# nanoporetech/vbz_compression

Hardware: AMD Instinct MI355X
Metric: MB/s encode+decode, int16 signal, 1/2/4/8 MI355X vs CPU; ratio preserved (higher is better)
Workload: dtype int16

## Files before the change

### vbz_compression_amd/csrc/vbz_api.hip

```cpp
#include <hip/hip_runtime.h>

#include <cmath>
#include <cstdarg>
#include <cstdio>
#include <cstdlib>
#include <cstring>
#include <condition_variable>
#include <mutex>
#include <string>
#include <map>
#include <vector>

#include "../../include/vbz.h"
#include "../../include/vbz_gpu.h"
#include "vbz_kernels.h"

using namespace vbzhip;


struct ProfEntry
{
    const char* name;
    uint32_t launches;
    double ms;
// ... 152 lines not shown

void drain_profile(vbz_gpu_ctx* c)
{
    if (c->pending.empty()) return;
    (void)hipStreamSynchronize(c->stream);
    for (auto& p : c->pending) {
        float ms = 0;
        (void)hipEventElapsedTime(&ms, p.start, p.stop);
        bool found = false;
        for (auto& e : c->prof)
            if (e.name == p.name || strcmp(e.name, p.name) == 0) {
                e.launches++;
                e.ms += ms;
                found = true;
                break;
            }
        if (!found) c->prof.push_back({ p.name, 1, (double)ms });
        c->event_pool.push_back(p.start);
        c->event_pool.push_back(p.stop);
    }
    c->pending.clear();
}

unsigned long long* dbg_begin(vbz_gpu_ctx* c, uint32_t n)
{
    if (!c->phase_timing) return nullptr;
    if (!ensure(c, c->dbg, (size_t)n * PHASE_SLOTS * 8)) return nullptr;
    (void)hipMemsetAsync(c->dbg.p, 0, (size_t)n * PHASE_SLOTS * 8, c->stream);
    return (unsigned long long*)c->dbg.p;
}

void dbg_end(vbz_gpu_ctx* c, uint32_t n, const char* what, unsigned long long* d)
{
    if (!d) return;
    std::vector<unsigned long long> h((size_t)n * PHASE_SLOTS);
    (void)hipStreamSynchronize(c->stream);
    (void)hipMemcpy(h.data(), d, (size_t)n * PHASE_SLOTS * 8, hipMemcpyDeviceToHost);
    double sum[PHASE_SLOTS] = {};
    for (uint32_t i = 0; i < n; ++i)
        for (int k = 0; k < PHASE_SLOTS; ++k) sum[k] += (double)h[(size_t)i * PHASE_SLOTS + k];
    fprintf(stderr, "vbz_hip phase cycles/read (%s, n=%u):", what, n);
    for (int k = 0; k < PHASE_SLOTS; ++k) fprintf(stderr, " p%d=%.0f", k, sum[k] / n);
    fprintf(stderr, "\n");
}

bool half_codec(const CompressionOptions* o) { return o->vbz_version == 1 && o->integer_size == 1; }

bool pod5_codec(const CompressionOptions* o) { return o->vbz_version == VBZ_GPU_VERSION_POD5; }

bool valid_int_size(const CompressionOptions* o)
{
    return o->integer_size == 0 || o->integer_size == 1 || o->integer_size == 2 || o->integer_size == 4;
}

bool batch_options_ok(const CompressionOptions* o, int sized)
{
    if (pod5_codec(o)) return o->integer_size == 2 && o->perform_delta_zig_zag && o->zstd_compression_level >= 1 && sized == 0;
// ... 205 lines not shown
            gate = pre->gate;
            scratch_planned = true;
        }
    }
    void* const scratch_base = pre ? pre->scratch : c->scratch.p;
    const ScratchPlan splan = { num, den, c->scratch.cap, svb_off, svb_cap, gate };
    if (segmented && plan_segments(c, n, bt->src_size, rb_in.gate, bt->src_bytes, svb_seg_unit_bytes((int)o->integer_size), &seg,
                                   both_stages ? &splan : nullptr, &scratch_planned) != 0)
        return -1;
    if (segmented) rb.gate = seg.gate;
    if (o->integer_size != 0 && o->zstd_compression_level == 0) {
        Timed t(c, "svb_encode");
        if (segmented)
            HIPCHK(c, launch_svb_encode_seg(rb, (int)o->integer_size, o->perform_delta_zig_zag, hdr, true, seg.first, seg.max_segs, seg.val, seg.off, s),
                   "svb_encode (segmented) launch");
        else
            HIPCHK(c, launch_svb_encode(rb, (int)o->integer_size, o->perform_delta_zig_zag, hdr, true, half_codec(o), nullptr, nullptr, s), "svb_encode launch");
        return 0;
    }
    if (o->integer_size == 0) {
        if (checksum_content(c, rb, rb.gate) != 0) return -1;
        {
            Timed t(c, "zstd_encode");
            HIPCHK(c, launch_zstd_encode(rb, bt->src_size, 0, nullptr, hdr, nullptr, nullptr, nullptr, c->trailers, nullptr, nullptr, false, false, nullptr, s), "zstd_encode launch");
        }
        return checksum_frames(c, rb, rb.gate, hdr, bt->src_size, 0);
    }
    const bool matcher = !segmented && c->zero_run_sequences && c->long_repeats;
    if (!scratch_planned) {
        if (rb.gate) HIPCHK(c, hipMemcpyAsync(gate, rb.gate, 4ull * n, hipMemcpyDeviceToDevice, s), "gate copy");
        Timed t(c, "plan_scratch");
        HIPCHK(c, launch_plan_scratch(n, bt->src_size, num, den, c->scratch.cap, svb_off, svb_cap, gate, rb.gate != nullptr, s), "plan launch");
    }
    ReadBatch a = rb;
    a.dst = (uint8_t*)scratch_base;
    a.dst_off = svb_off;
    a.dst_cap = svb_cap;
    a.result = svb_size;
    a.gate = gate;
    unsigned long long* dbg = segmented ? nullptr : dbg_begin(c, n);
    const bool staged = !segmented && c->staged_encode && (!dbg || c->phase_timing == 3) && c->zero_run_sequences;
    const bool pod5 = pod5_codec(o);
    const bool pre_filled = staged && !pod5 && svb_encode_fills_plans((int)o->integer_size, o->perform_delta_zig_zag, half_codec(o));
    void* plan = nullptr;
    if (staged) {
        if (!ensure(c, c->encplan, zstd_encode_plan_bytes(n))) return -1;
        plan = c->encplan.p;
    }
    const uint32_t* key_orig = bt->src_size;
    uint32_t key_elem = o->integer_size;
    if (pod5) {
        HIPCHK(c, launch_svb16_key_raw(n, bt->src_size, key_raw, s), "svb16 key launch");
        key_orig = key_raw;
        key_elem = SVB16_KEY_ELEM;
    }
    {
        Timed t(c, "svb_encode");
        if (pod5)
            HIPCHK(c, launch_svb16_encode(a, (matcher && !segmented) ? deep_d : nullptr, s), "svb16_encode launch");
        else if (segmented)
            HIPCHK(c, launch_svb_encode_seg(a, (int)o->integer_size, o->perform_delta_zig_zag, 0, false, seg.first, seg.max_segs, seg.val, seg.off, s),
                   "svb_encode (segmented) launch");
        else
            HIPCHK(c, launch_svb_encode(a, (int)o->integer_size, o->perform_delta_zig_zag, 0, false, half_codec(o), matcher ? deep_d : nullptr,
// ... 22 lines not shown
        uint32_t* span_first = sm.take<uint32_t>((size_t)n + 1);
        uint32_t* span_count = sm.take<uint32_t>(1);
        uint32_t* span_size = sm.take<uint32_t>(max_spans);
        uint32_t* span_trail = sm.take<uint32_t>(max_spans);
        uint32_t* span_dst = sm.take<uint32_t>(max_spans);
        z.gate = gate;
        if (c->zero_run_sequences && c->long_repeats && o->integer_size != 0) {
            uint32_t* gate2 = mc.take<uint32_t>(n);
            Timed t(c, "zstd_encode_matcher");
            HIPCHK(c, launch_zstd_encode_matcher(z, key_orig, key_elem, hdr, svb_cap, c->seqtab.p, c->trailers, 0xFFFFFFFFu,
                                                 deep_d, gate, gate2, s),
                   "zstd_encode (matcher) launch");
            z.gate = gate2;
        }
        Timed t(c, "zstd_encode");
        HIPCHK(c, launch_zstd_encode_spans(z, key_orig, key_elem, hdr, c->zero_run_sequences ? svb_cap : nullptr,
                                           c->zero_run_sequences ? c->seqtab.p : nullptr, desc, span_first, span_count, max_spans,
                                           (uint8_t*)c->spantmp.p, tmp_bytes, span_size, span_trail, span_dst, c->trailers, regions, shspan, s),
               "zstd_encode (spans) launch");
        return checksum_frames(c, z, gate, hdr, pod5 ? nullptr : bt->src_size, o->integer_size);
    }
    {
        Timed t(c, "zstd_encode");
        HIPCHK(c, launch_zstd_encode(z, key_orig, key_elem, nullptr, hdr, c->phase_timing == 3 ? nullptr : dbg,
                                     c->zero_run_sequences ? svb_cap : nullptr, c->zero_run_sequences ? c->seqtab.p : nullptr, c->trailers,
                                     (matcher && !dbg) ? deep_d : nullptr, plan, staged, pre_filled, c->phase_timing == 3 ? dbg : nullptr, s),
               "zstd_encode launch");
    }
    dbg_end(c, n,
            c->phase_timing == 3   ? "zstd_pack: setup region lookups+scan bits quads ends+headers sequences trailer"
            : c->phase_timing == 2 ? "zstd_encode planning launch: setup hist plan - store+sequences - | plan: sort merge lengths codes weights tree"
                                   : "zstd_encode: setup hist plan size hdr encode",
            dbg);
    return checksum_frames(c, z, gate, hdr, pod5 ? nullptr : bt->src_size, o->integer_size);
}

constexpr uint32_t REF_MIN_READS = 2560;

int zstd_frames(vbz_gpu_ctx* c, const ReadBatch& z, uint32_t toosmall_code, uint64_t content_bytes, unsigned long long* dbg)
{
    const uint32_t n = z.n_reads;
    hipStream_t s = c->stream;
    Timed t(c, "zstd_decode");
    c->last_frames = 0;
    if (!c->fast_decode) {
        HIPCHK(c, launch_zstd_decode(z, toosmall_code, dbg, c->seqdtab.p, s), "zstd_decode launch");
        return 0;
    }
    if (!ensure(c, c->fastmeta, zstd_fast_meta_bytes(n))) return -1;
    const bool walk = (c->ref_chains >= 2 || (c->ref_chains == 1 && n >= REF_MIN_READS)) && (c->foreign_state != 0 || c->ref_chains >= 2);
    const uint64_t recs_bytes = walk ? std::min<uint64_t>(((content_bytes >> 2) + (1ull << 20)) & ~15ull, 1ull << 30) : 0;
    if (walk && (!ensure(c, c->refpre, zstd_ref_pre_bytes(n)) || !ensure(c, c->reftab, zstd_ref_table_bytes(n)) || !ensure(c, c->refrecs, recs_bytes)))
        return -1;
    if (walk && !dbg && !ensure_side(c)) return -1;
    const bool lits = walk && zstd_ref_literals_enabled();
    if (lits && !ensure(c, c->reflits, zstd_ref_lit_meta_bytes(n))) return -1;
// ... 914 lines not shown
        if (integer_size != 2 || !zigzag) return -2;
        Timed t(c, "svb_decode");
        HIPCHK(c, launch_svb16_decode(to_rb(bt), c->stream), "svb16_decode launch");
        return 0;
    }
    if ((integer_size != 1 && integer_size != 2 && integer_size != 4) || version > 1 || version < 0) return -2;
    Timed t(c, "svb_decode");
    HIPCHK(c, launch_svb_decode(to_rb(bt), integer_size, zigzag != 0, version == 1 && integer_size == 1, c->stream), "svb_decode launch");
    return 0;
}

uint64_t vbz_gpu_pod5_max_compressed_size(uint32_t samples)
{
    const uint64_t n = samples, svb = (n + 7) / 8 + 2 * n;
    return svb + (svb >> 8) + (svb < (128u << 10) ? (((128u << 10) - svb) >> 11) : 0);
}

int vbz_gpu_zstd_compress_batch(vbz_gpu_ctx* c, const vbz_gpu_batch* bt, const uint32_t* key_bytes)
{
    if (!c || !bt) return -1;
    DeviceGuard dg(c->device);
    if (checksum_content(c, to_rb(bt), nullptr) != 0) return -1;
    Timed t(c, "zstd_encode");
    HIPCHK(c, launch_zstd_encode(to_rb(bt), bt->src_size, 0, key_bytes, 0, nullptr, nullptr, nullptr, c->trailers, nullptr, nullptr, false, false, nullptr, c->stream), "zstd_encode launch");
    return checksum_frames(c, to_rb(bt), nullptr, 0, nullptr, 0);
}

int vbz_gpu_zstd_decompress_batch(vbz_gpu_ctx* c, const vbz_gpu_batch* bt)
{
    if (!c || !bt) return -1;
    DeviceGuard dg(c->device);
    if (!plausible_extents(c, bt)) return -2;
    if (zstd_frames(c, to_rb(bt), E_ZSTD, bt->dst_bytes, nullptr) != 0) return -1;
    return verify_checksums(c, to_rb(bt));
}

int vbz_gpu_xxh64_batch(vbz_gpu_ctx* c, const vbz_gpu_batch* bt, uint64_t* out)
{
    if (!c || !bt || !out) return -1;
    DeviceGuard dg(c->device);
    Timed t(c, "xxh64");
    HIPCHK(c, launch_xxh64_batch((const uint8_t*)bt->src, bt->src_off, bt->src_size, nullptr, nullptr, bt->n_reads, out, c->stream), "xxh64 launch");
    return 0;
}

static bool pack_align_ok(vbz_gpu_ctx* c, uint32_t align)
{
// ... 573 lines not shown
```

### vbz_compression_amd/csrc/vbz_kernels.h

```cpp
#pragma once

#include <hip/hip_runtime.h>
#include <stdint.h>

namespace vbzhip {

constexpr uint32_t E_ZSTD = 0xFFFFFFFFu;
constexpr uint32_t E_INPUT_SIZE = 0xFFFFFFFEu;
constexpr uint32_t E_INTEGER_SIZE = 0xFFFFFFFDu;
constexpr uint32_t E_DESTINATION_SIZE = 0xFFFFFFFCu;
constexpr uint32_t E_STREAM = 0xFFFFFFFBu;
constexpr uint32_t E_VERSION = 0xFFFFFFFAu;
constexpr uint32_t E_OOM = 0xFFFFFFF9u;
constexpr uint32_t E_DEVICE = 0xFFFFFFF8u;
constexpr uint32_t E_FIRST = E_DEVICE;
constexpr uint32_t GATE_SKIP = E_FIRST - 1u;
constexpr int PHASE_SLOTS = 12;

constexpr uint32_t SIG_NONE = 0, SIG_F32 = 1, SIG_F16 = 2, SIG_BF16 = 3;
constexpr uint32_t SIG_CHUNK = 4;
constexpr uint32_t SIG_COUNT = 8;
constexpr uint32_t CHUNK_PAD = 0, CHUNK_END = 1;

constexpr uint32_t NORM_MED_MAD = 1, NORM_QUANTILE = 2;
// ... 78 lines not shown
    uint32_t pad[8];
    uint32_t histB[256];
};
constexpr uint32_t PLAN_OPEN = 1, PLAN_REG0 = 2, PLAN_REG1 = 4, PLAN_READY = 7;
constexpr uint32_t ENC_TRAILERS = 1, ENC_PRE_FILLED = 2;
inline EncPlan* zstd_encode_plans(void* plan_meta) { return reinterpret_cast<EncPlan*>(plan_meta); }

hipError_t launch_svb_encode(const ReadBatch& b, int integer_size, bool zigzag, uint32_t hdr, bool strict_cap, bool half, uint32_t* period_hint,
                             void* plans, hipStream_t s);
bool svb_encode_fills_plans(int integer_size, bool zigzag, bool half);
hipError_t launch_svb_decode(const ReadBatch& b, int integer_size, bool zigzag, bool half, hipStream_t s);
hipError_t launch_svb16_encode(const ReadBatch& b, uint32_t* period_hint, hipStream_t s);
hipError_t launch_svb16_decode(const ReadBatch& b, hipStream_t s);
hipError_t launch_svb16_key_raw(uint32_t n, const uint32_t* raw_size, uint32_t* key_raw, hipStream_t s);
constexpr uint32_t SVB16_KEY_ELEM = 4;
uint32_t svb_seg_unit_bytes(int integer_size);
hipError_t launch_svb_encode_seg(const ReadBatch& b, int integer_size, bool zigzag, uint32_t hdr, bool strict_cap, const uint32_t* seg_first,
                                 uint32_t max_segs, uint32_t* seg_bytes, uint64_t* seg_off, hipStream_t s);
hipError_t launch_svb_decode_seg(const ReadBatch& b, int integer_size, bool zigzag, const uint32_t* seg_first, uint32_t max_segs,
                                 uint32_t* seg_val, uint64_t* seg_pos, uint32_t* seg_run, hipStream_t s);

hipError_t launch_zstd_encode(const ReadBatch& b, const uint32_t* orig_size, uint32_t key_elem, const uint32_t* key_bytes,
                              uint32_t hdr, unsigned long long* dbg, const uint32_t* src_cap, const void* seq_tables, bool trailers,
                              uint32_t* deep_d, void* plan_meta, bool staged, bool pre_filled, unsigned long long* pack_dbg, hipStream_t s);
size_t zstd_encode_plan_bytes(uint32_t n_reads);
size_t seq_tables_bytes();
void seq_tables_build(void* host_buffer);
struct SideStream
{
    hipStream_t stream = nullptr;
    hipEvent_t fork = nullptr, join = nullptr;
};
typedef SideStream FastSide;
size_t zstd_span_desc_bytes();
uint32_t zstd_span_max_spans(uint64_t stream_bytes, uint32_t n_reads);
uint64_t zstd_span_tmp_bytes(uint64_t stream_bytes, uint32_t n_reads, uint32_t max_spans);
hipError_t launch_zstd_encode_spans(const ReadBatch& b, const uint32_t* orig_size, uint32_t key_elem, uint32_t hdr, const uint32_t* src_cap,
                                    const void* seq_tables, void* span_desc, uint32_t* span_first, uint32_t* span_count, uint32_t max_spans,
                                    uint8_t* span_tmp, uint64_t span_tmp_bytes, uint32_t* span_size, uint32_t* span_trail, uint32_t* span_dst,
                                    bool trailers, void* shared_regions, uint32_t shared_span_bytes, hipStream_t s);
size_t zstd_span_region_bytes(uint32_t n_reads);
uint32_t zstd_span_shared_bytes(uint64_t stream_bytes);
hipError_t launch_zstd_encode_matcher(const ReadBatch& b, const uint32_t* orig_size, uint32_t key_elem, uint32_t hdr, const uint32_t* src_cap,
                                      const void* seq_tables, bool trailers, uint32_t max_raw, uint32_t* deep_d, const uint32_t* gate_in,
                                      uint32_t* gate_out, hipStream_t s);
hipError_t launch_zstd_decode(const ReadBatch& b, uint32_t toosmall_code, unsigned long long* dbg, const void* seq_dtables,
                              hipStream_t s);
// ... 163 lines not shown
```

### vbz_compression_amd/csrc/zstd_encode.hip

```cpp
#include "vbz_kernels.h"
#include "zstd_entropy.h"
#include "zstd_frame.h"

namespace vbzhip {

namespace {

constexpr int WAVE = 64;
constexpr uint32_t BLOCK_MAX = 128u << 10;
constexpr uint32_t MIN_BLOCK = 4096;
constexpr uint32_t HUF_BLOCK_MAX = 92u << 10;
constexpr uint32_t SPLIT_MIN = 2048;
constexpr int MAXBLK = 16;
#ifndef VBZ_SPAN_BLOCK_KB
#define VBZ_SPAN_BLOCK_KB 16
#endif
constexpr uint32_t SPAN_BLOCK = VBZ_SPAN_BLOCK_KB << 10;
#ifndef VBZ_SPAN_SMALL_BLOCKS
#define VBZ_SPAN_SMALL_BLOCKS 2
#endif
constexpr uint32_t SPAN_BYTES_SMALL = SPAN_BLOCK * VBZ_SPAN_SMALL_BLOCKS, SPAN_BYTES_LARGE = SPAN_BLOCK * MAXBLK;
constexpr uint32_t SPAN_LARGE_FROM = 256u << 20;
#ifndef VBZ_KEYSPAN_KB
#define VBZ_KEYSPAN_KB 8
// ... 57 lines not shown
    uint32_t mode;
    uint32_t huffLog;
    uint32_t rankcnt[16];
    union
    {
        HufPmWksp pm;
        FseWeightWksp fw;
        struct
        {
            uint32_t ssize[WAVE];
            uint32_t sbeg[WAVE];
            uint32_t scnt[WAVE];
            uint32_t obuf[OBUF_WORDS];
            uint16_t seqcode[8 + 256];
            uint32_t seqpiece[256];
        };
    };
    SeqCTables seq;
    uint32_t cp[64];
    uint32_t cpCount, cpSpacing;
    __device__ __forceinline__ void set_code(uint32_t s, uint32_t code, uint32_t nb) { ctable[s] = make_uint2(code, nb); }
};

struct TableLds
{
    uint32_t hist[256];
    uint32_t ctable[256];
    uint8_t nbBits[256];
    uint8_t weights[260];
    uint8_t tree[136];
    int32_t treeSize;
    uint32_t mode;
    uint32_t huffLog;
    uint32_t rankcnt[16];
    union
    {
        HufPmWksp pm;
        FseWeightWksp fw;
    };
    __device__ __forceinline__ void set_code(uint32_t s, uint32_t code, uint32_t nb) { ctable[s] = code | (nb << 16); }
};
struct TokSeqLds
{
    uint32_t obuf[128];
    uint16_t seqcode[8 + 256];
    uint32_t seqpiece[256];
    SeqCTables seq;
    uint32_t cp[64];
    uint32_t cpCount, cpSpacing;
};

__device__ __forceinline__ void put_le(uint8_t* p, uint64_t v, int n)
{
    for (int i = 0; i < n; ++i) {
        uint32_t byte = (uint32_t)(v >> (8 * i)) & 0xFFu;
        asm volatile("" : "+v"(byte));
        p[i] = (uint8_t)byte;
    }
}

__device__ __forceinline__ uint32_t wave_sum_u32(uint32_t v)
// ... 35 lines not shown
{
    uint32_t seen = 0;
    uint32_t c[4];
#pragma unroll
    for (int j = 0; j < 4; ++j) {
        c[j] = sample[lane + 64 * j];
        seen += c[j] ? 1u : 0u;
    }
    seen = wave_sum_u32(seen);
    if (allow_sample && n >= HIST_SAMPLE_FROM && seen >= HIST_SAMPLE_SEEN) {
#pragma unroll
        for (int j = 0; j < 4; ++j) L.hist[lane + 64 * j] = c[j] ? c[j] : 1u;
        wave_lds_sync();
        return hist_sample_bytes(in, n) + (256u - seen);
    }
    if (!rest) return region_histogram(L, in, n, lane, allow_sample);
#pragma unroll
    for (int j = 0; j < 4; ++j) L.hist[lane + 64 * j] = c[j] + rest[lane + 64 * j];
    wave_lds_sync();
    return n;
}

template <class LDS>
__device__ __forceinline__ uint32_t region_histogram(LDS& L, const uint8_t* in, uint32_t n, int lane, bool allow_sample)
{
    static_assert(sizeof(HufPmWksp) >= 4 * 256 * sizeof(uint32_t), "the sub-histograms live in the table-construction workspace");
    uint32_t* sub = reinterpret_cast<uint32_t*>(&L.pm);
    for (int i = lane; i < 4 * 256; i += WAVE) sub[i] = 0;
    wave_lds_sync();
    uint32_t* mine = sub + 256 * (lane & 3);
    const uint32_t head = (uint32_t)((16u - ((uintptr_t)in & 15u)) & 15u);
    const uint32_t h = head < n ? head : n;
    if ((uint32_t)lane < h) atomicAdd(&mine[in[lane]], 1u);
    const uint32_t nvec = (n - h) >> 4;
    const uint4* vp = reinterpret_cast<const uint4*>(in + h);
    const uint32_t tail0 = h + (nvec << 4);
    if (tail0 + (uint32_t)lane < n) atomicAdd(&mine[in[tail0 + lane]], 1u);
    auto count = [&](uint32_t first_stripe, uint32_t stripe_step, uint32_t trip_stripes, int loads) {
        for (uint32_t s0 = first_stripe; s0 * WAVE < nvec; s0 += trip_stripes) {
            uint4 q[4];
#pragma unroll
            for (int u = 0; u < 4; ++u) {
                const uint32_t c = (s0 + (uint32_t)u * stripe_step) * WAVE + (uint32_t)lane;
                q[u] = (u < loads && c < nvec) ? vp[c] : make_uint4(0u, 0u, 0u, 0u);
            }
#pragma unroll
            for (int u = 0; u < 4; ++u) {
                const uint32_t c = (s0 + (uint32_t)u * stripe_step) * WAVE + (uint32_t)lane;
                if (u < loads && c < nvec) {
                    const uint32_t w[4] = { q[u].x, q[u].y, q[u].z, q[u].w };
// ... 30 lines not shown
        count(1, 1, 4, 3);
    } else {
        count(0, 1, 4, 4);
    }
    (void)total();
    return n;
}

#define SUB(k) do { if (tsub) { unsigned long long tn = __builtin_readcyclecounter(); tsub[k] += tn - *tl; *tl = tn; } } while (0)
template <bool STRICT>
__device__ __forceinline__ uint32_t sorted_count(const uint32_t* arr, uint32_t v, uint32_t top)
{
    uint32_t lo = 0;
    for (uint32_t step = top; step; step >>= 1) {
        const uint32_t x = arr[lo + step - 1];
        lo += (STRICT ? x < v : x <= v) ? step : 0u;
    }
    return lo;
}

template <class LDS>
__device__ __forceinline__ uint32_t huf_build_wave(LDS& L, uint32_t maxSym, uint32_t maxNbBits, int lane, unsigned long long* tsub = nullptr, unsigned long long* tl = nullptr)
{
    HufPmWksp& K = L.pm;
    uint32_t key[4];
    {
        const uint4 h = *reinterpret_cast<const uint4*>(&L.hist[4 * lane]);
        const uint32_t c[4] = { h.x, h.y, h.z, h.w };
#pragma unroll
        for (int j = 0; j < 4; ++j) {
            const uint32_t sy = 4u * (uint32_t)lane + (uint32_t)j;
            key[j] = (sy <= maxSym && c[j]) ? ((c[j] << 8) | (255u - sy)) : 0xFFFFFFFFu;
        }
    }
    for (int i = lane; i < (HUF_MAX_BITS + 1) * 16; i += WAVE) (&K.isPkg[0][0])[i] = 0;
#pragma unroll
    for (int k = 2; k <= 256; k <<= 1) {
#pragma unroll
        for (int d = k >> 1; d > 0; d >>= 1) {
            if (d >= 4) {
                const int m = d >> 2;
                const bool up = ((4 * lane) & k) == 0, lower = (lane & m) == 0;
                const bool keep_min = lower == up;
#pragma unroll
                for (int j = 0; j < 4; ++j) {
                    const uint32_t o = (uint32_t)__shfl_xor((int)key[j], m, 64);
                    const uint32_t mn = o < key[j] ? o : key[j], mx = o < key[j] ? key[j] : o;
                    key[j] = keep_min ? mn : mx;
                }
            } else {
#pragma unroll
                for (int a = 0; a < 4; ++a) {
                    const int bb = a ^ d;
                    if (bb > a) {
                        const bool up = ((4 * lane + a) & k) == 0;
                        const uint32_t mn = key[a] < key[bb] ? key[a] : key[bb], mx = key[a] < key[bb] ? key[bb] : key[a];
                        key[a] = up ? mn : mx;
                        key[bb] = up ? mx : mn;
// ... 22 lines not shown
    const uint32_t X0 = 2u * n - 2u;
    const uint32_t nj = (n + 63u) >> 6;
    constexpr uint32_t PM_INF = 0xFFFFFFFFu;
    uint32_t ln[4] = { 0, 0, 0, 0 };
    uint32_t lk[8];
    {
        uint4 a = make_uint4(PM_INF, PM_INF, PM_INF, PM_INF), c = a;
        if (lane < 32) {
            a = *reinterpret_cast<const uint4*>(&K.leaf[8 * lane]);
            c = *reinterpret_cast<const uint4*>(&K.leaf[8 * lane + 4]);
        }
        const uint32_t w8[8] = { a.x, a.y, a.z, a.w, c.x, c.y, c.z, c.w };
#pragma unroll
        for (int r = 0; r < 8; ++r) lk[r] = w8[r] == PM_INF ? PM_INF : w8[r] << 1;
    }
    uint32_t m = n >> 1;
    uint32_t pk4[4];
#pragma unroll
    for (int q = 0; q < 4; ++q) {
        const uint32_t t = 4u * (uint32_t)lane + (uint32_t)q;
        pk4[q] = t < m ? ((((lk[2 * q] >> 1) + (lk[2 * q + 1] >> 1)) << 1) | 1u) : PM_INF;
    }
    wave_lds_sync();
    uint64_t* const masks = reinterpret_cast<uint64_t*>(K.merged);
    uint32_t levSame = maxNbBits;
    for (uint32_t lev = 2; lev <= maxNbBits; ++lev) {
        const bool last = lev == maxNbBits;
        uint32_t it[8];
        {
            const int src = 2 * (63 - lane);
#pragma unroll
            for (int r = 0; r < 8; ++r) {
                const uint32_t p = (uint32_t)__shfl((int)pk4[(7 - r) & 3], (src + ((7 - r) >> 2)) & 63, 64);
                it[r] = lane < 32 ? lk[r] : p;
            }
        }
#pragma unroll
        for (int dl = 32; dl >= 1; dl >>= 1) {
            const bool lower = (lane & dl) == 0;
#pragma unroll
            for (int r = 0; r < 8; ++r) {
                const uint32_t o = (uint32_t)__shfl_xor((int)it[r], dl, 64);
                const uint32_t mn = o < it[r] ? o : it[r], mx = o < it[r] ? it[r] : o;
                it[r] = lower ? mn : mx;
            }
        }
#pragma unroll
// ... 309 lines not shown
    while (span * 2 <= r) { w &= w >> span; span *= 2; }
    if (span < r) w &= w >> (r - span);
    return w;
}

__device__ __forceinline__ uint64_t dilate_left(uint64_t w, uint32_t r)
{
    uint32_t span = 1;
    while (span * 2 <= r) { w |= w << span; span *= 2; }
    if (span < r) w |= w << (r - span);
    return w;
}

constexpr uint32_t RPER = 16;
template <bool PERIOD, bool COUNT_ONLY = false, bool TSUB = false>
__device__ void tokenise_runs(uint8_t* k, uint32_t K, uint2* rec, uint32_t& Lit, uint32_t& nrec, const uint16_t* mask16, int lane,
                              unsigned long long* tsub_ = nullptr, unsigned long long* tl = nullptr)
{
    unsigned long long* const tsub = TSUB ? tsub_ : nullptr;
    uint32_t lit_total = 0, rec_total = 0;
    uint32_t carry60 = 0, carry61 = 0;
    uint32_t carryw = 0;
    const uint64_t below = (1ull << lane) - 1ull;
    for (uint32_t pb = 0; pb < K; pb += TOK_PAYLOAD) {
        const int64_t lo = (int64_t)pb + 16 * ((int64_t)lane - 2);
        uint32_t w[4] = { 0, 0, 0, 0 };
        uint32_t zm = 0, valid = 0;
        if (lane >= 2 && lo < (int64_t)K) {
            uint4 v;
            __builtin_memcpy(&v, k + lo, 16);
            w[0] = v.x; w[1] = v.y; w[2] = v.z; w[3] = v.w;
            const uint32_t nvalid = (K - (uint32_t)lo) >= 16 ? 16u : (K - (uint32_t)lo);
            valid = nvalid >= 16 ? 0xFFFFu : ((1u << nvalid) - 1u);
        }
        if (PERIOD) {
            zm = (lane >= 2 && lo < (int64_t)K) ? (uint32_t)mask16[(uint32_t)lo >> 4] & valid : 0u;
        } else {
            uint32_t pw = wave_prev_lane_u32(w[3]);
            if (lane == 2) pw = carryw;
#pragma unroll
            for (int q = 0; q < 4; ++q) {
                const uint32_t x = w[q] ^ __builtin_amdgcn_alignbyte(w[q], q ? w[q - 1] : pw, 3);
                const uint32_t z = ~(((x & 0x7F7F7F7Fu) + 0x7F7F7F7Fu) | x) & 0x80808080u;
                zm |= ((((z >> 7) * 0x00204081u) >> 21) & 0xFu) << (4 * q);
            }
            zm &= valid;
            if (lane == 2 && pb == 0) zm &= ~1u;
        }
        if (!PERIOD) {
            if (lane == 0) zm = carry60;
            if (lane == 1) zm = carry61;
        } else if (lane < 2) {
            const int64_t lb = (int64_t)pb + 16 * ((int64_t)lane - 2);
            zm = lb >= 0 ? (uint32_t)mask16[(uint32_t)lb >> 4] : 0u;
// ... 1077 lines not shown
                put_le(tp + 8, L.cpSpacing | (count << 16), 4);
                put_le(tp + 12 + 4 * count, tb, 4);
            }
            if ((uint32_t)lane < count) put_le(tp + 12 + 4 * lane, L.cp[lane], 4);
            opos += tb;
        }
    }
    if (span_mode) {
        if (lane == 0) {
            span_size[blockIdx.x] = main_bytes;
            span_trail[blockIdx.x] = opos - main_bytes;
        }
    } else if (lane == 0) {
        b.result[r] = opos;
    }
    if (TIMED && lane == 0 && !span_mode)
        for (int k = 0; k < PHASE_SLOTS; ++k) dbg[(size_t)r * PHASE_SLOTS + k] = tph[k];
#undef PHASE
#undef NEED
#undef FINISH
}

#ifndef VBZ_TABLE_WAVES
#define VBZ_TABLE_WAVES 5
#endif

__device__ __forceinline__ uint32_t enc_key_bytes(uint32_t N, uint32_t r, const uint32_t* orig_size, uint32_t key_elem, const uint32_t* key_bytes)
{
    uint32_t K = 0;
    if (N >= SPLIT_MIN) {
        if (key_bytes) K = key_bytes[r];
        else if (key_elem) K = (orig_size[r] / key_elem + 3u) >> 2;
        if (K >= N) K = 0;
    }
    return K;
}
__device__ __forceinline__ uint32_t enc_block_target(uint32_t N)
{
    const uint32_t T = (N + 13) / 14;
    return T < MIN_BLOCK ? MIN_BLOCK : (T > HUF_BLOCK_MAX ? HUF_BLOCK_MAX : T);
}

__device__ __forceinline__ bool plan_guess_tokenised(uint32_t N, uint32_t K) { return K != 0 ? (K >= 256 && K <= BLOCK_MAX) : (N >= 256 && N <= BLOCK_MAX); }

struct PlanLds
{
    union
    {
        TokSeqLds ts;
        TableLds tb;
    };
};

__device__ __forceinline__ bool plan_region_table(TableLds& L, EncPlan* FP, uint32_t region, const uint8_t* rin, uint32_t S, uint32_t nblk, bool seqmode,
                                                  uint32_t nrec, bool from_plan, int lane)
{
    uint32_t Sh;
    if (from_plan) Sh = region_histogram_from_plan(L, rin, S, lane, true, FP->reg[1].ctable, FP->hist_mode == 2u ? FP->histB : nullptr);
    else Sh = region_histogram(L, rin, S, lane, !seqmode);
    region_plan(L, S, Sh, nblk, lane);
    wave_lds_sync();
    if (L.mode != 2u) return false;
    EncRegionPlan* P = &FP->reg[region];
#pragma unroll
    for (int j = 0; j < 4; ++j) P->ctable[lane + 64 * j] = L.ctable[lane + 64 * j];
    if (lane < 34) P->tree[lane] = reinterpret_cast<const uint32_t*>(L.tree)[lane];
    if (lane == 0) {
        P->S = S;
        P->nblk = nblk;
        P->nrec = nrec;
        P->seqmode = seqmode ? 1u : 0u;
        P->Sh = Sh;
        P->treeSize = (uint32_t)L.treeSize;
        P->huffLog = L.huffLog;
    }
    return nblk <= (uint32_t)MAXBLK;
}

__global__ __launch_bounds__(WAVE, VBZ_TABLE_WAVES) void zstd_plan_kernel(ReadBatch b, const uint32_t* orig_size, uint32_t key_elem, const uint32_t* key_bytes,
                                                                          uint32_t hdr, const uint32_t* src_cap, const SeqCTables* seqtab, uint32_t* deep_d,
                                                                          EncPlan* plans, uint32_t* pstate, uint32_t pre_filled)
{
    __shared__ __attribute__((aligned(16))) PlanLds LL;
    const int lane = threadIdx.x;
    const uint32_t r = blockIdx.x >> 1, role = blockIdx.x & 1u;
    EncPlan* FP = &plans[r];
    if (role == 0 && lane == 0) {
        FP->tok_done = 0;
        FP->seqBytes = 0;
        FP->seqOff = 0;
        FP->cpCount = 0;
        FP->cpSpacing = 0;
    }
    if (b.gate && b.gate[r] >= GATE_SKIP) return;
    const uint32_t N = b.src_size[r];
    if (N >= E_FIRST || N == 0) return;
    const uint8_t* in = b.src + b.src_off[r];
    const uint32_t K = enc_key_bytes(N, r, orig_size, key_elem, key_bytes);
    const uint32_t T = enc_block_target(N);
    const bool guess = src_cap && seqtab && plan_guess_tokenised(N, K);
    if (role == 1) {
        if (K == 0) return;
        uint32_t S = N - K;
        uint32_t nblk = (S + T - 1) / T;
        if (guess) {
            uint32_t Td = (S + DATA_BLOCKS - 1) / DATA_BLOCKS;
            Td = Td < MIN_BLOCK ? MIN_BLOCK : (Td > HUF_BLOCK_MAX ? HUF_BLOCK_MAX : Td);
            nblk = (S + Td - 1) / Td;
        }
        const bool ok = plan_region_table(LL.tb, FP, 1, in + K, S, nblk, false, 0, pre_filled && FP->hist_mode != 0, lane);
        __syncthreads();
        if (ok && lane == 0) atomicOr(&pstate[r], PLAN_REG1);
        return;
    }
    const uint32_t cap = b.dst_cap[r];
    uint8_t* out = b.dst + b.dst_off[r];
    if (deep_d) {
        uint32_t hint = deep_d[r];
        if (hint) {
            bool ok = false;
            if (K != 0 && src_cap && seqtab && N - K >= 8192) {
                DeepLayout dl;
                if (hint == RUN_D) hint = run_period(in + K, N - K, lane);
                ok = deep_layout(N, K, in, src_cap[r], out, cap, hdr, dl) && period_holds(in + K, N - K, hint, lane);
            }
            if (lane == 0) deep_d[r] = ok ? hint : 0u;
            if (ok) return;
        }
    }
    if ((uint64_t)hdr + 9 > cap) return;
    const uint32_t S0 = K ? K : N;
    uint32_t nrec = 0, Lit = 0;
    const uint2* rec = nullptr;
    if (src_cap && seqtab && S0 >= 256 && S0 <= BLOCK_MAX) {
        const uint32_t slot = src_cap[r];
        const uint32_t recs_all = S0 / RMIN + 2u + 2u;
        const uint64_t need = (uint64_t)N + 16 + 8ull * recs_all;
        if (need <= slot) {
            uint8_t* ws = const_cast<uint8_t*>(in) + ((slot - 8u * recs_all) & ~7u);
            tokenise_runs<false>(const_cast<uint8_t*>(in), S0, reinterpret_cast<uint2*>(ws), Lit, nrec, nullptr, lane);
            __syncthreads();
            rec = reinterpret_cast<const uint2*>(ws);
            if (lane == 0) {
                FP->tok_nrec = nrec;
                FP->tok_lit = Lit;
                FP->tok_done = 1;
            }
        }
    }
    if ((nrec != 0) != guess) return;
    if (nrec) {
        const uint64_t room = 24ull + 8ull * nrec;
        if (room + 4096u > cap) return;
        const uint32_t so = (uint32_t)((cap - room) & ~15ull);
        TokSeqLds& L = LL.ts;
        {
            const uint32_t* g = reinterpret_cast<const uint32_t*>(seqtab);
            uint32_t* l = reinterpret_cast<uint32_t*>(&L.seq);
            for (uint32_t i = lane; i < sizeof(SeqCTables) / 4; i += WAVE) l[i] = g[i];
        }
        wave_lds_sync();
        const uint32_t sb = encode_zero_run_sequences(L, out + so, rec, nrec, lane, 0u);
        wave_lds_sync();
        FP->cp[lane] = L.cp[lane];
        if (lane == 0) {
            FP->seqBytes = sb;
            FP->seqOff = so;
            FP->cpCount = L.cpCount;
            FP->cpSpacing = L.cpSpacing;
        }
        wave_lds_sync();
    }
    const uint32_t S = nrec ? Lit : S0;
    const uint32_t nblk = nrec ? 1u : (S + T - 1) / T;
    const bool ok = plan_region_table(LL.tb, FP, 0, in, S, nblk, nrec != 0, nrec, false, lane);
    __syncthreads();
    if (ok && lane == 0) atomicOr(&pstate[r], PLAN_OPEN | PLAN_REG0 | (K == 0 ? PLAN_REG1 : 0u));
}

#ifndef VBZ_PACK_TABLE_COPIES
#define VBZ_PACK_TABLE_COPIES 1
#endif
constexpr int PACK_COPIES = VBZ_PACK_TABLE_COPIES;
struct PackLds
{
    uint32_t ctable[PACK_COPIES * 256];
    uint32_t tree[34];
    uint32_t ssize[WAVE], sbeg[WAVE], scnt[WAVE];
    uint32_t obuf[2][OBUF_WORDS];
};

template <bool TIMED>
__device__ __forceinline__ bool pack_region(PackLds& L, const uint8_t* rin, uint32_t r0, uint8_t* out, uint32_t& opos, uint32_t limit, const uint32_t* ctable_g,
                                            const uint32_t* tree_g, uint32_t S, uint32_t nblk, uint32_t treeSize, bool seqmode, bool lastRegion,
                                            uint32_t seqBytes, uint32_t seqOff, int lane, unsigned long long (&tph)[PHASE_SLOTS], unsigned long long& tlast)
{
#define PPHASE(k) do { if (TIMED) { unsigned long long tn = __builtin_readcyclecounter(); tph[k] += tn - tlast; tlast = tn; } } while (0)
#define REDO() return false
    wave_lds_sync();
#pragma unroll
    for (int j = 0; j < 4; ++j) {
// ... 674 lines not shown
        }
    }
    __syncthreads();
    if (tid < WAVE) {
        const uint32_t hint = best == 0xFFFFFFFFu ? ((!placed && SD >= PP_P0 + PP_TRIES * PP_SHIFT + 48u) ? RUN_D : 0u) : best;
        uint32_t D = 0;
        if (hint) {
            const uint8_t* in = b.src + b.src_off[r];
            DeepLayout dl;
            const uint32_t h2 = hint == RUN_D ? run_period(in + K, SD, tid) : hint;
            if (deep_layout(N, K, in, src_cap[r], b.dst + b.dst_off[r], b.dst_cap[r], hdr, dl) && period_holds(in + K, SD, h2, tid)) D = h2;
        }
        if (tid == 0) {
            deep_d[r] = D;
            gate_out[r] = D ? GATE_SKIP : (gate ? gate[r] : 0u);
        }
    }
}

}

hipError_t launch_zstd_encode(const ReadBatch& b, const uint32_t* orig_size, uint32_t key_elem, const uint32_t* key_bytes,
                              uint32_t hdr, unsigned long long* dbg, const uint32_t* src_cap, const void* seq_tables, bool trailers,
                              uint32_t* deep_d, void* plan_meta, bool staged, bool pre_filled, unsigned long long* pack_dbg, hipStream_t s)
{
    if (!plan_meta) staged = pre_filled = false;
    const uint32_t tr = (trailers ? ENC_TRAILERS : 0u) | (pre_filled ? ENC_PRE_FILLED : 0u);
    if (b.n_reads == 0) return hipSuccess;
    const SeqCTables* st = reinterpret_cast<const SeqCTables*>(seq_tables);
#ifdef VBZ_EXPERIMENTS
    if (dbg && !plan_meta) {
        hipLaunchKernelGGL((zstd_encode_kernel<true, false>), dim3(b.n_reads), dim3(WAVE), 0, s, b, orig_size, key_elem, key_bytes, hdr, dbg,
                           src_cap, st, nullptr, nullptr, nullptr, nullptr, nullptr, tr, nullptr, nullptr, nullptr, SpanShared{});
        return hipGetLastError();
    }
#else
    dbg = nullptr;
    pack_dbg = nullptr;
#endif
    EncPlan* plans = reinterpret_cast<EncPlan*>(plan_meta);
    uint32_t* redo = plans ? reinterpret_cast<uint32_t*>(plans + b.n_reads) : nullptr;
    if (staged && src_cap && st) {
        (void)hipMemsetAsync(redo, 0, 4ull * b.n_reads, s);
        hipLaunchKernelGGL(zstd_plan_kernel, dim3(2 * b.n_reads), dim3(WAVE), 0, s, b, orig_size, key_elem, key_bytes, hdr, src_cap, st, deep_d, plans, redo,
                           pre_filled ? 1u : 0u);
#ifdef VBZ_EXPERIMENTS
        if (pack_dbg)
            hipLaunchKernelGGL(zstd_pack_kernel<true>, dim3(b.n_reads), dim3(WAVE), 0, s, b, orig_size, key_elem, key_bytes, hdr, tr, plans, redo, pack_dbg);
        else
#endif
        hipLaunchKernelGGL(zstd_pack_kernel<false>, dim3(b.n_reads), dim3(WAVE), 0, s, b, orig_size, key_elem, key_bytes, hdr, tr, plans, redo, (unsigned long long*)nullptr);
    } else {
        redo = nullptr;
    }
    hipLaunchKernelGGL((zstd_encode_kernel<false, false>), dim3(b.n_reads), dim3(WAVE), 0, s, b, orig_size, key_elem, key_bytes, hdr, nullptr,
                       src_cap, st, nullptr, nullptr, nullptr, nullptr, nullptr, tr, deep_d, redo ? plans : nullptr, redo, SpanShared{});
    if (deep_d)
        hipLaunchKernelGGL((zstd_encode_kernel<false, true>), dim3(b.n_reads), dim3(WAVE), 0, s, b, orig_size, key_elem, key_bytes, hdr, nullptr,
                           src_cap, st, nullptr, nullptr, nullptr, nullptr, nullptr, tr, deep_d, redo ? plans : nullptr, nullptr, SpanShared{});
    return hipGetLastError();
}

size_t zstd_encode_plan_bytes(uint32_t n_reads) { return (size_t)n_reads * (sizeof(EncPlan) + 4) + 256; }

hipError_t launch_zstd_encode_matcher(const ReadBatch& b, const uint32_t* orig_size, uint32_t key_elem, uint32_t hdr, const uint32_t* src_cap,
                                      const void* seq_tables, bool trailers, uint32_t max_raw, uint32_t* deep_d, const uint32_t* gate_in,
                                      uint32_t* gate_out, hipStream_t s)
{
// ... 58 lines not shown
```

Measured before the change: 613,400.

## Shrink plan-kernel LDS, raise table-wave occupancy, prefetch tokeniser loads, add plan timing

The table-construction LDS is reorganised so the sub-histograms overlay the ctable/tree fields and the package-merge workspace is replaced by a smaller per-wave layout, and VBZ_TABLE_WAVES goes from 5 to 7. Together these aim to let more plan-kernel waves stay resident per CU. The tokeniser loop now issues the next 16-byte load one iteration ahead to hide global-memory latency. It also adds per-role phase timing instrumentation for the plan kernel, which only compiles in under VBZ_EXPERIMENTS. The risk is register pressure at the higher launch bound and correctness of the overlaid LDS lifetimes, including the removed zeroing of the package flags.

```diff
diff --git a/vbz_compression_amd/csrc/vbz_api.hip b/vbz_compression_amd/csrc/vbz_api.hip
--- a/vbz_compression_amd/csrc/vbz_api.hip
+++ b/vbz_compression_amd/csrc/vbz_api.hip
@@ -198,17 +198,40 @@
     c->pending.clear();
 }
 
-unsigned long long* dbg_begin(vbz_gpu_ctx* c, uint32_t n)
+unsigned long long* dbg_begin(vbz_gpu_ctx* c, uint32_t n, bool per_role = false)
 {
     if (!c->phase_timing) return nullptr;
+    if (per_role) n *= 2;
     if (!ensure(c, c->dbg, (size_t)n * PHASE_SLOTS * 8)) return nullptr;
     (void)hipMemsetAsync(c->dbg.p, 0, (size_t)n * PHASE_SLOTS * 8, c->stream);
     return (unsigned long long*)c->dbg.p;
 }
 
-void dbg_end(vbz_gpu_ctx* c, uint32_t n, const char* what, unsigned long long* d)
+void dbg_end_roles(vbz_gpu_ctx* c, uint32_t n, const char* what, unsigned long long* d)
+{
+    std::vector<unsigned long long> h((size_t)n * PHASE_SLOTS);
+    (void)hipStreamSynchronize(c->stream);
+    (void)hipMemcpy(h.data(), d, (size_t)n * PHASE_SLOTS * 8, hipMemcpyDeviceToHost);
+    for (uint32_t role = 0; role < 2; ++role) {
+        double sum[PHASE_SLOTS] = {};
+        uint32_t m = 0;
+        for (uint32_t i = role; i < n; i += 2) {
+            unsigned long long t = 0;
+            for (int k = 0; k < PHASE_SLOTS; ++k) t += h[(size_t)i * PHASE_SLOTS + k];
+            if (!t) continue;
+            ++m;
+            for (int k = 0; k < PHASE_SLOTS; ++k) sum[k] += (double)h[(size_t)i * PHASE_SLOTS + k];
+        }
+        fprintf(stderr, "vbz_hip phase cycles/read (%s, role %u, n=%u):", what, role, m);
+        for (int k = 0; k < PHASE_SLOTS; ++k) fprintf(stderr, " p%d=%.0f", k, m ? sum[k] / m : 0.0);
+        fprintf(stderr, "\n");
+    }
+}
+
+void dbg_end(vbz_gpu_ctx* c, uint32_t n, const char* what, unsigned long long* d, bool per_role = false)
 {
     if (!d) return;
+    if (per_role) return dbg_end_roles(c, 2 * n, what, d);
     std::vector<unsigned long long> h((size_t)n * PHASE_SLOTS);
     (void)hipStreamSynchronize(c->stream);
     (void)hipMemcpy(h.data(), d, (size_t)n * PHASE_SLOTS * 8, hipMemcpyDeviceToHost);
@@ -460,7 +483,7 @@
         if (checksum_content(c, rb, rb.gate) != 0) return -1;
         {
             Timed t(c, "zstd_encode");
-            HIPCHK(c, launch_zstd_encode(rb, bt->src_size, 0, nullptr, hdr, nullptr, nullptr, nullptr, c->trailers, nullptr, nullptr, false, false, nullptr, s), "zstd_encode launch");
+            HIPCHK(c, launch_zstd_encode(rb, bt->src_size, 0, nullptr, hdr, nullptr, nullptr, nullptr, c->trailers, nullptr, nullptr, false, false, nullptr, nullptr, s), "zstd_encode launch");
         }
         return checksum_frames(c, rb, rb.gate, hdr, bt->src_size, 0);
     }
@@ -476,8 +499,8 @@
     a.dst_cap = svb_cap;
     a.result = svb_size;
     a.gate = gate;
-    unsigned long long* dbg = segmented ? nullptr : dbg_begin(c, n);
-    const bool staged = !segmented && c->staged_encode && (!dbg || c->phase_timing == 3) && c->zero_run_sequences;
+    unsigned long long* dbg = segmented ? nullptr : dbg_begin(c, n, c->phase_timing == 2);
+    const bool staged = !segmented && c->staged_encode && (!dbg || c->phase_timing == 2 || c->phase_timing == 3) && c->zero_run_sequences;
     const bool pod5 = pod5_codec(o);
     const bool pre_filled = staged && !pod5 && svb_encode_fills_plans((int)o->integer_size, o->perform_delta_zig_zag, half_codec(o));
     void* plan = nullptr;
@@ -546,16 +569,18 @@
     }
     {
         Timed t(c, "zstd_encode");
-        HIPCHK(c, launch_zstd_encode(z, key_orig, key_elem, nullptr, hdr, c->phase_timing == 3 ? nullptr : dbg,
+        const bool staged_timing = c->phase_timing == 2 || c->phase_timing == 3;
+        HIPCHK(c, launch_zstd_encode(z, key_orig, key_elem, nullptr, hdr, staged_timing ? nullptr : dbg,
                                      c->zero_run_sequences ? svb_cap : nullptr, c->zero_run_sequences ? c->seqtab.p : nullptr, c->trailers,
-                                     (matcher && !dbg) ? deep_d : nullptr, plan, staged, pre_filled, c->phase_timing == 3 ? dbg : nullptr, s),
+                                     (matcher && !dbg) ? deep_d : nullptr, plan, staged, pre_filled, c->phase_timing == 2 ? dbg : nullptr,
+                                     c->phase_timing == 3 ? dbg : nullptr, s),
                "zstd_encode launch");
     }
     dbg_end(c, n,
             c->phase_timing == 3   ? "zstd_pack: setup region lookups+scan bits quads ends+headers sequences trailer"
-            : c->phase_timing == 2 ? "zstd_encode planning launch: setup hist plan - store+sequences - | plan: sort merge lengths codes weights tree"
+            : c->phase_timing == 2 ? "zstd_plan: setup tokeniser sequences hist store rest | sort merge leaves lengths codes+weights tree"
                                    : "zstd_encode: setup hist plan size hdr encode",
-            dbg);
+            dbg, c->phase_timing == 2);
     return checksum_frames(c, z, gate, hdr, pod5 ? nullptr : bt->src_size, o->integer_size);
 }
 
@@ -1516,7 +1541,7 @@
     DeviceGuard dg(c->device);
     if (checksum_content(c, to_rb(bt), nullptr) != 0) return -1;
     Timed t(c, "zstd_encode");
-    HIPCHK(c, launch_zstd_encode(to_rb(bt), bt->src_size, 0, key_bytes, 0, nullptr, nullptr, nullptr, c->trailers, nullptr, nullptr, false, false, nullptr, c->stream), "zstd_encode launch");
+    HIPCHK(c, launch_zstd_encode(to_rb(bt), bt->src_size, 0, key_bytes, 0, nullptr, nullptr, nullptr, c->trailers, nullptr, nullptr, false, false, nullptr, nullptr, c->stream), "zstd_encode launch");
     return checksum_frames(c, to_rb(bt), nullptr, 0, nullptr, 0);
 }
 
diff --git a/vbz_compression_amd/csrc/vbz_kernels.h b/vbz_compression_amd/csrc/vbz_kernels.h
--- a/vbz_compression_amd/csrc/vbz_kernels.h
+++ b/vbz_compression_amd/csrc/vbz_kernels.h
@@ -124,7 +124,8 @@
 
 hipError_t launch_zstd_encode(const ReadBatch& b, const uint32_t* orig_size, uint32_t key_elem, const uint32_t* key_bytes,
                               uint32_t hdr, unsigned long long* dbg, const uint32_t* src_cap, const void* seq_tables, bool trailers,
-                              uint32_t* deep_d, void* plan_meta, bool staged, bool pre_filled, unsigned long long* pack_dbg, hipStream_t s);
+                              uint32_t* deep_d, void* plan_meta, bool staged, bool pre_filled, unsigned long long* plan_dbg, unsigned long long* pack_dbg,
+                              hipStream_t s);
 size_t zstd_encode_plan_bytes(uint32_t n_reads);
 size_t seq_tables_bytes();
 void seq_tables_build(void* host_buffer);
diff --git a/vbz_compression_amd/csrc/zstd_encode.hip b/vbz_compression_amd/csrc/zstd_encode.hip
--- a/vbz_compression_amd/csrc/zstd_encode.hip
+++ b/vbz_compression_amd/csrc/zstd_encode.hip
@@ -103,21 +103,35 @@
     __device__ __forceinline__ void set_code(uint32_t s, uint32_t code, uint32_t nb) { ctable[s] = make_uint2(code, nb); }
 };
 
+struct HufPmWave
+{
+    uint32_t leaf[256];
+    uint8_t sym[256];
+};
+static_assert(sizeof(HufPmWave::leaf) >= 8 * 8 * (HUF_MAX_BITS + 1), "the package masks ([level][8] x 64 bits) fit in the leaves' place");
+
 struct TableLds
 {
     uint32_t hist[256];
-    uint32_t ctable[256];
-    uint8_t nbBits[256];
-    uint8_t weights[260];
-    uint8_t tree[136];
-    int32_t treeSize;
-    uint32_t mode;
-    uint32_t huffLog;
-    uint32_t rankcnt[16];
     union
     {
-        HufPmWksp pm;
-        FseWeightWksp fw;
+        uint32_t sub[4 * 256];
+        struct
+        {
+            uint32_t ctable[256];
+            uint8_t nbBits[256];
+            uint8_t weights[260];
+            uint8_t tree[136];
+            int32_t treeSize;
+            uint32_t mode;
+            uint32_t huffLog;
+            uint32_t rankcnt[16];
+            union
+            {
+                HufPmWave pm;
+                FseWeightWksp fw;
+            };
+        };
     };
     __device__ __forceinline__ void set_code(uint32_t s, uint32_t code, uint32_t nb) { ctable[s] = code | (nb << 16); }
 };
@@ -199,10 +213,17 @@
 }
 
 template <class LDS>
+__device__ __forceinline__ uint32_t* hist_subs(LDS& L)
+{
+    static_assert(sizeof(L.pm) >= 4 * 256 * sizeof(uint32_t), "the sub-histograms live in the table-construction workspace");
+    return reinterpret_cast<uint32_t*>(&L.pm);
+}
+__device__ __forceinline__ uint32_t* hist_subs(TableLds& L) { return L.sub; }
+
+template <class LDS>
 __device__ __forceinline__ uint32_t region_histogram(LDS& L, const uint8_t* in, uint32_t n, int lane, bool allow_sample)
 {
-    static_assert(sizeof(HufPmWksp) >= 4 * 256 * sizeof(uint32_t), "the sub-histograms live in the table-construction workspace");
-    uint32_t* sub = reinterpret_cast<uint32_t*>(&L.pm);
+    uint32_t* sub = hist_subs(L);
     for (int i = lane; i < 4 * 256; i += WAVE) sub[i] = 0;
     wave_lds_sync();
     uint32_t* mine = sub + 256 * (lane & 3);
@@ -279,7 +300,7 @@
 template <class LDS>
 __device__ __forceinline__ uint32_t huf_build_wave(LDS& L, uint32_t maxSym, uint32_t maxNbBits, int lane, unsigned long long* tsub = nullptr, unsigned long long* tl = nullptr)
 {
-    HufPmWksp& K = L.pm;
+    auto& K = L.pm;
     uint32_t key[4];
     {
         const uint4 h = *reinterpret_cast<const uint4*>(&L.hist[4 * lane]);
@@ -290,7 +311,6 @@
             key[j] = (sy <= maxSym && c[j]) ? ((c[j] << 8) | (255u - sy)) : 0xFFFFFFFFu;
         }
     }
-    for (int i = lane; i < (HUF_MAX_BITS + 1) * 16; i += WAVE) (&K.isPkg[0][0])[i] = 0;
 #pragma unroll
     for (int k = 2; k <= 256; k <<= 1) {
 #pragma unroll
@@ -359,7 +379,7 @@
         pk4[q] = t < m ? ((((lk[2 * q] >> 1) + (lk[2 * q + 1] >> 1)) << 1) | 1u) : PM_INF;
     }
     wave_lds_sync();
-    uint64_t* const masks = reinterpret_cast<uint64_t*>(K.merged);
+    uint64_t* const masks = reinterpret_cast<uint64_t*>(K.leaf);
     uint32_t levSame = maxNbBits;
     for (uint32_t lev = 2; lev <= maxNbBits; ++lev) {
         const bool last = lev == maxNbBits;
@@ -715,14 +735,19 @@
     uint32_t carry60 = 0, carry61 = 0;
     uint32_t carryw = 0;
     const uint64_t below = (1ull << lane) - 1ull;
+    auto request = [&](uint32_t pb_) {
+        uint4 v = make_uint4(0u, 0u, 0u, 0u);
+        const int64_t lo_ = (int64_t)pb_ + 16 * ((int64_t)lane - 2);
+        if (lane >= 2 && lo_ < (int64_t)K) __builtin_memcpy(&v, k + lo_, 16);
+        return v;
+    };
+    uint4 next = request(0);
     for (uint32_t pb = 0; pb < K; pb += TOK_PAYLOAD) {
         const int64_t lo = (int64_t)pb + 16 * ((int64_t)lane - 2);
-        uint32_t w[4] = { 0, 0, 0, 0 };
+        uint32_t w[4] = { next.x, next.y, next.z, next.w };
+        if (pb + TOK_PAYLOAD < K) next = request(pb + TOK_PAYLOAD);
         uint32_t zm = 0, valid = 0;
         if (lane >= 2 && lo < (int64_t)K) {
-            uint4 v;
-            __builtin_memcpy(&v, k + lo, 16);
-            w[0] = v.x; w[1] = v.y; w[2] = v.z; w[3] = v.w;
             const uint32_t nvalid = (K - (uint32_t)lo) >= 16 ? 16u : (K - (uint32_t)lo);
             valid = nvalid >= 16 ? 0xFFFFu : ((1u << nvalid) - 1u);
         }
@@ -1846,7 +1871,7 @@
 }
 
 #ifndef VBZ_TABLE_WAVES
-#define VBZ_TABLE_WAVES 5
+#define VBZ_TABLE_WAVES 7
 #endif
 
 __device__ __forceinline__ uint32_t enc_key_bytes(uint32_t N, uint32_t r, const uint32_t* orig_size, uint32_t key_elem, const uint32_t* key_bytes)
@@ -1876,13 +1901,17 @@
     };
 };
 
+#define PT(k) do { if (TIMED) { const unsigned long long tn_ = __builtin_readcyclecounter(); tph[k] += tn_ - tlast; tlast = tn_; } } while (0)
+
+template <bool TIMED>
 __device__ __forceinline__ bool plan_region_table(TableLds& L, EncPlan* FP, uint32_t region, const uint8_t* rin, uint32_t S, uint32_t nblk, bool seqmode,
-                                                  uint32_t nrec, bool from_plan, int lane)
+                                                  uint32_t nrec, bool from_plan, int lane, unsigned long long* tph, unsigned long long& tlast)
 {
     uint32_t Sh;
     if (from_plan) Sh = region_histogram_from_plan(L, rin, S, lane, true, FP->reg[1].ctable, FP->hist_mode == 2u ? FP->histB : nullptr);
     else Sh = region_histogram(L, rin, S, lane, !seqmode);
-    region_plan(L, S, Sh, nblk, lane);
+    PT(3);
+    region_plan(L, S, Sh, nblk, lane, TIMED ? tph : nullptr, &tlast);
     wave_lds_sync();
     if (L.mode != 2u) return false;
     EncRegionPlan* P = &FP->reg[region];
@@ -1898,16 +1927,25 @@
         P->treeSize = (uint32_t)L.treeSize;
         P->huffLog = L.huffLog;
     }
+    PT(4);
     return nblk <= (uint32_t)MAXBLK;
 }
 
+template <bool TIMED>
 __global__ __launch_bounds__(WAVE, VBZ_TABLE_WAVES) void zstd_plan_kernel(ReadBatch b, const uint32_t* orig_size, uint32_t key_elem, const uint32_t* key_bytes,
                                                                           uint32_t hdr, const uint32_t* src_cap, const SeqCTables* seqtab, uint32_t* deep_d,
-                                                                          EncPlan* plans, uint32_t* pstate, uint32_t pre_filled)
+                                                                          EncPlan* plans, uint32_t* pstate, uint32_t pre_filled, unsigned long long* dbg)
 {
     __shared__ __attribute__((aligned(16))) PlanLds LL;
     const int lane = threadIdx.x;
     const uint32_t r = blockIdx.x >> 1, role = blockIdx.x & 1u;
+    unsigned long long tph[TIMED ? PHASE_SLOTS : 1] = {};
+    unsigned long long tlast = TIMED ? __builtin_readcyclecounter() : 0ull;
+    auto timed_out = [&]() {
+        PT(5);
+        if (TIMED && lane == 0)
+            for (int k = 0; k < PHASE_SLOTS; ++k) dbg[(size_t)blockIdx.x * PHASE_SLOTS + k] = tph[k];
+    };
     EncPlan* FP = &plans[r];
     if (role == 0 && lane == 0) {
         FP->tok_done = 0;
@@ -1932,9 +1970,11 @@
             Td = Td < MIN_BLOCK ? MIN_BLOCK : (Td > HUF_BLOCK_MAX ? HUF_BLOCK_MAX : Td);
             nblk = (S + Td - 1) / Td;
         }
-        const bool ok = plan_region_table(LL.tb, FP, 1, in + K, S, nblk, false, 0, pre_filled && FP->hist_mode != 0, lane);
+        PT(0);
+        const bool ok = plan_region_table<TIMED>(LL.tb, FP, 1, in + K, S, nblk, false, 0, pre_filled && FP->hist_mode != 0, lane, tph, tlast);
         __syncthreads();
         if (ok && lane == 0) atomicOr(&pstate[r], PLAN_REG1);
+        timed_out();
         return;
     }
     const uint32_t cap = b.dst_cap[r];
@@ -1962,8 +2002,10 @@
         const uint64_t need = (uint64_t)N + 16 + 8ull * recs_all;
         if (need <= slot) {
             uint8_t* ws = const_cast<uint8_t*>(in) + ((slot - 8u * recs_all) & ~7u);
+            PT(0);
             tokenise_runs<false>(const_cast<uint8_t*>(in), S0, reinterpret_cast<uint2*>(ws), Lit, nrec, nullptr, lane);
             __syncthreads();
+            PT(1);
             rec = reinterpret_cast<const uint2*>(ws);
             if (lane == 0) {
                 FP->tok_nrec = nrec;
@@ -1994,13 +2036,17 @@
             FP->cpSpacing = L.cpSpacing;
         }
         wave_lds_sync();
+        PT(2);
     }
     const uint32_t S = nrec ? Lit : S0;
     const uint32_t nblk = nrec ? 1u : (S + T - 1) / T;
-    const bool ok = plan_region_table(LL.tb, FP, 0, in, S, nblk, nrec != 0, nrec, false, lane);
+    PT(0);
+    const bool ok = plan_region_table<TIMED>(LL.tb, FP, 0, in, S, nblk, nrec != 0, nrec, false, lane, tph, tlast);
     __syncthreads();
     if (ok && lane == 0) atomicOr(&pstate[r], PLAN_OPEN | PLAN_REG0 | (K == 0 ? PLAN_REG1 : 0u));
-}
+    timed_out();
+}
+#undef PT
 
 #ifndef VBZ_PACK_TABLE_COPIES
 #define VBZ_PACK_TABLE_COPIES 1
@@ -2721,7 +2767,8 @@
 
 hipError_t launch_zstd_encode(const ReadBatch& b, const uint32_t* orig_size, uint32_t key_elem, const uint32_t* key_bytes,
                               uint32_t hdr, unsigned long long* dbg, const uint32_t* src_cap, const void* seq_tables, bool trailers,
-                              uint32_t* deep_d, void* plan_meta, bool staged, bool pre_filled, unsigned long long* pack_dbg, hipStream_t s)
+                              uint32_t* deep_d, void* plan_meta, bool staged, bool pre_filled, unsigned long long* plan_dbg, unsigned long long* pack_dbg,
+                              hipStream_t s)
 {
     if (!plan_meta) staged = pre_filled = false;
     const uint32_t tr = (trailers ? ENC_TRAILERS : 0u) | (pre_filled ? ENC_PRE_FILLED : 0u);
@@ -2735,14 +2782,21 @@
     }
 #else
     dbg = nullptr;
+    plan_dbg = nullptr;
     pack_dbg = nullptr;
 #endif
     EncPlan* plans = reinterpret_cast<EncPlan*>(plan_meta);
     uint32_t* redo = plans ? reinterpret_cast<uint32_t*>(plans + b.n_reads) : nullptr;
     if (staged && src_cap && st) {
         (void)hipMemsetAsync(redo, 0, 4ull * b.n_reads, s);
-        hipLaunchKernelGGL(zstd_plan_kernel, dim3(2 * b.n_reads), dim3(WAVE), 0, s, b, orig_size, key_elem, key_bytes, hdr, src_cap, st, deep_d, plans, redo,
-                           pre_filled ? 1u : 0u);
+#ifdef VBZ_EXPERIMENTS
+        if (plan_dbg)
+            hipLaunchKernelGGL(zstd_plan_kernel<true>, dim3(2 * b.n_reads), dim3(WAVE), 0, s, b, orig_size, key_elem, key_bytes, hdr, src_cap, st, deep_d, plans,
+                               redo, pre_filled ? 1u : 0u, plan_dbg);
+        else
+#endif
+        hipLaunchKernelGGL(zstd_plan_kernel<false>, dim3(2 * b.n_reads), dim3(WAVE), 0, s, b, orig_size, key_elem, key_bytes, hdr, src_cap, st, deep_d, plans,
+                           redo, pre_filled ? 1u : 0u, (unsigned long long*)nullptr);
 #ifdef VBZ_EXPERIMENTS
         if (pack_dbg)
             hipLaunchKernelGGL(zstd_pack_kernel<true>, dim3(b.n_reads), dim3(WAVE), 0, s, b, orig_size, key_elem, key_bytes, hdr, tr, plans, redo, pack_dbg);
```

After: 624,200 (median of 6 runs). 1.02x the previous value.
